# HySonLab/Protein_Redesign

Hardware: AMD Instinct MI355X
Metric: denoising-steps/sec (fwd+rev) per complex, N=256 res (higher is better)
Workload: dtype f32; 1 GPU; configs[1]: synthetic 256-residue + 64-atom ligand (N=320), single_dim=512 pair_dim=64 num_blocks=4 num_steps=1000, 1 complex/GPU, sharded by sample index (no data-path collective; one all_gather of the samples at the end of the timed region); samples_per_gpu=1, hip_graph=True, outputs_finite=True, backend=single process

## Files before the change

include/prd_hip.h:

```cpp
#ifndef PRD_HIP_H
#define PRD_HIP_H

#include <stddef.h>
#include <stdint.h>

#ifdef __cplusplus
extern "C" {
#endif

#ifndef __HIP__
typedef struct ihipStream_t* hipStream_t;
#endif

#define PRD_VERSION 101
#define PRD_STEP_BOUNDARY_SYNC_INTS 2
#define PRD_ERR_ARG (-1)
#define PRD_ERR_ALIGN (-2)
#define PRD_ERR_UNSUPPORTED (-3)
#define PRD_ERR_WORKSPACE (-4)

int prd_version(void);

#define PRD_ARITH_FP32 0
#define PRD_ARITH_SPLIT16 1
// ... 29 lines not shown
    int act, act_from;
    const float* addmat; long long sad1, sad2; int ldadd;
    const float* colmask; long long scm1; float fill;
    const float* rowmask; long long srm1;
    const float* mulmat; long long smu1, smu2; int ldmul;
    const float* resid; long long sr1, sr2; int ldr;
    int tile_hint;
    int a_ln;
    float* ln_out; int ldlo;
    int arith;
    float* C2; int ldc2; int n_split;
    int rowmask_cols;
    const float* rscale;
    float* ws; size_t ws_bytes;
    const float* wsum;
    float* out_ln; int ldol;
    float a_scale;
    int mul_pos;
    const unsigned* a_amax;
} PrdGemm;
size_t prd_gemm_slab_workspace(int M, int N, int K);
int prd_gemm_slab_ok(int M, int N, int K, int arith);
int prd_gemm(const PrdGemm* args, hipStream_t stream);

int prd_ln_rows(const float* x, float* y, const float* gamma, const float* beta,
                int rows, int C, int ldx, int ldy, hipStream_t stream);
int prd_softmax_rows(float* x, int rows, int n, int ld, hipStream_t stream);

int prd_static_pair(float* out, const float* atom_mask, const float* residue_mask, const float* bond_mask,
                    const int64_t* bond_feats, const int64_t* bond_distance,
                    const int64_t* residue_index, const int64_t* chain_index,
                    const float* tab_b0, const float* tab_b1, const float* tab_b2,
                    const float* tab_bdist, const float* tab_relpos,
                    int max_bond_distance, int max_relpos, int b, int N, int P, hipStream_t stream);
int prd_atom_embed(float* out, const int64_t* atom_feats, const float* atom_mask, const float* tables,
                   const int* offsets, int n_feats, int b, int N, int S, hipStream_t stream);
int prd_single_init(float* single, const float* static_single, const float* seq_t, const float* residue_mask,
                    const float* w_rt, int rows, int S, int n_cls, hipStream_t stream);
int prd_time_embed(float* ebeta, const int64_t* t, const float* freqs, const float* w_beta,
                   int num_steps, int b, int P, int time_dim, hipStream_t stream);
int prd_pair_init(float* pair, const float* static_pair, const float* z, const float* mask,
                  const float* centers, const float* w_dist, const float* ebeta,
                  int b, int N, int P, int dist_dim, int arith, hipStream_t stream);

int prd_pair_bias(float* bias_out, const float* pair, const float* gamma, const float* beta,
                  const float* w, const float* bvec, int b, int N, int P, int H, hipStream_t stream);
// ... 143 lines not shown
```

protein_redesign_amd/_lib.py:

```python
from __future__ import annotations

import ctypes as C
import os

import torch

HERE = os.path.dirname(os.path.abspath(__file__))
LIB_PATH = os.environ.get("PRD_LIB", os.path.join(HERE, "libprd_hip.so"))

vp, ci, cf, cz, cll = C.c_void_p, C.c_int, C.c_float, C.c_size_t, C.c_longlong


class PrdGemm(C.Structure):
    _fields_ = [
        ("A", vp), ("B", vp), ("C", vp),
        ("M", ci), ("N", ci), ("K", ci),
        ("lda", ci), ("ldb", ci), ("ldc", ci),
        ("G1", ci), ("G2", ci),
        ("sa1", cll), ("sa2", cll), ("sb1", cll), ("sb2", cll), ("sc1", cll), ("sc2", cll),
        ("b_kn", ci), ("alpha", cf), ("colscale", vp),
        ("bias", vp), ("act", ci), ("act_from", ci),
        ("addmat", vp), ("sad1", cll), ("sad2", cll), ("ldadd", ci),
        ("colmask", vp), ("scm1", cll), ("fill", cf),
        ("rowmask", vp), ("srm1", cll),
# ... 1 lines not shown
        ("resid", vp), ("sr1", cll), ("sr2", cll), ("ldr", ci),
        ("tile_hint", ci),
        ("a_ln", ci),
        ("ln_out", vp), ("ldlo", ci),
        ("arith", ci),
        ("C2", vp), ("ldc2", ci), ("n_split", ci),
        ("rowmask_cols", ci),
        ("rscale", vp),
        ("ws", vp), ("ws_bytes", cz),
        ("wsum", vp),
        ("out_ln", vp), ("ldol", ci),
        ("a_scale", cf),
        ("mul_pos", ci),
        ("a_amax", vp),
    ]


SIGNATURES = {
    "prd_version": [],
    "prd_tri_attn_variant": [ci, ci, ci],
    "prd_gemm": [C.POINTER(PrdGemm), vp],
    "prd_gemm_slab_workspace": [ci, ci, ci],
    "prd_gemm_slab_ok": [ci, ci, ci, ci],
    "prd_ln_rows": [vp, vp, vp, vp, ci, ci, ci, ci, vp],
    "prd_softmax_rows": [vp, ci, ci, ci, vp],
    "prd_static_pair": [vp] * 13 + [ci] * 5 + [vp],
    "prd_atom_embed": [vp] * 5 + [ci] * 4 + [vp],
    "prd_single_init": [vp] * 5 + [ci] * 3 + [vp],
    "prd_time_embed": [vp] * 4 + [ci] * 4 + [vp],
    "prd_pair_init": [vp] * 7 + [ci] * 5 + [vp],
    "prd_pair_bias": [vp] * 6 + [ci] * 4 + [vp],
    "prd_pair_bias2": [vp] * 6 + [ci] + [vp] * 5 + [ci] * 4 + [vp],
    "prd_opm_pair": [vp] * 6 + [ci] * 6 + [vp],
    "prd_pair_head_supported": [ci, ci, ci, ci],
    "prd_pair_head": [vp] * 7 + [ci] + [vp] * 3 + [ci, ci] + [vp] * 5 + [ci] + [vp] * 5 + [ci] * 5 + [vp],
    "prd_outer_linear": [vp] * 4 + [ci] + [vp] * 2 + [ci] * 5 + [vp, ci, vp],
    "prd_tri_mul": [vp] * 11 + [ci] * 5 + [vp, cz, vp, ci, vp],
    "prd_tri_mul_contract": [vp, vp, ci, ci, ci, ci, vp],
    "prd_tri_mul_contract_scaled": [vp, vp, vp, ci, ci, ci, ci, vp],
    "prd_tri_mul_chain_supported": [ci, ci, ci],
    "prd_tri_attn_core_fused_supported": [ci, ci, ci],
    "prd_tri_attn_core_fused": [vp] * 12 + [ci] * 6 + [vp],
    "prd_tri_mul_chain": [vp, vp, vp, vp, ci, ci, ci, vp, cz, ci, vp],
    "prd_tri_mul_out_bwd": [vp] * 15 + [ci] * 4 + [vp],
    "prd_tri_mul_out_bwd_amax": [vp] * 15 + [ci] * 4 + [vp, vp],
    "prd_tri_mul_bwd_operands": [vp, vp, ci, ci, ci, vp],
# ... 32 lines not shown
    "prd_tri_attn_v2_supported": [ci, ci, ci],
    "prd_tri_attn_out": [vp] * 5 + [ci] * 4 + [vp, ci, vp],
    "prd_spa_attn_core_supported": [ci, ci, ci],
    "prd_spa_attn_core_workspace": [ci, ci, ci, ci],
    "prd_spa_attn_core": [vp, vp, ci, vp, vp, ci, ci, ci, ci, vp, cz, ci, vp],
    "prd_workspace_bytes": [C.c_char_p, ci, ci, ci, ci],
    "prd_tri_attn_pair_supported": [ci, ci, ci],
    "prd_tri_attn_pair": [vp, vp, vp, vp, vp, ci, ci, ci, ci, ci, vp, ci, vp],
    "prd_tri_attn_heads_supported": [ci] * 5,
    "prd_tri_attn_heads_workspace_bytes": [ci] * 5,
    "prd_tri_attn_core_heads": [vp] * 8 + [ci] * 6 + [vp, cz, ci, vp],
    "prd_tri_attn_core_heads_lse": [vp] * 9 + [ci] * 6 + [vp, cz, ci, vp],
    "prd_tri_attn_bwd_heads_supported": [ci] * 5,
    "prd_tri_attn_bwd_heads_workspace_bytes": [ci] * 5,
    "prd_tri_attn_bwd_core_heads": [vp] * 12 + [ci] * 6 + [vp, cz, ci, vp],
}

GEMM_MODES = {"fp32": 0, "split16": 1, "bf16x3": 1}
DEFAULT_GEMM_MODE = "split16"

_ARITH_BEFORE_STREAM = ("prd_coord_head", "prd_pair_head", "prd_pair_init", "prd_opm_pair", "prd_outer_linear", "prd_tri_mul", "prd_tri_mul_contract", "prd_tri_mul_contract_scaled", "prd_tri_mul_proj_bwd",
                        "prd_tri_attn", "prd_tri_attn_core", "prd_tri_attn_out", "prd_pair_transition", "prd_block_tail", "prd_tri_mul_chain",
                        "prd_linear_wgrad", "prd_pair_linear", "prd_spa_attn_core", "prd_tri_attn_pair",
                        "prd_tri_attn_core_heads", "prd_tri_attn_core_heads_lse", "prd_tri_attn_bwd_core_heads")
_ARITH_LAST = ("prd_tri_attn_variant", "prd_tri_mul_chain_supported", "prd_tri_attn_core_fused_supported", "prd_tri_attn_stats_bytes",
               "prd_gemm_slab_ok", "prd_pair_head_supported", "prd_pair_linear_supported", "prd_spa_attn_core_supported",
               "prd_tri_attn_pair_supported", "prd_tri_attn_heads_supported",
               "prd_tri_attn_bwd_heads_supported")
_TUNE_BEFORE_STREAM = ("prd_tri_attn_core_v2", "prd_tri_attn_core_v2_lse")
_TUNE_LAST = ("prd_tri_attn_v2_supported", "prd_tri_attn_v2_form")


def tune_from_env(env=None) -> int:
    env = os.environ if env is None else env

    def geti(name, default):
        v = env.get(name)
        return default if v is None or v == "" else int(v)

    t = geti("PRD_TA_VARIANT", 0) & 15
    if geti("PRD_TA2_V3", 1) == 0:
        t |= 1 << 4
    if geti("PRD_TA2_LONG", 1) == 0:
        t |= 1 << 5
    f = geti("PRD_TA2_FLAGS", -1)
    if f >= 0:
        t |= (1 << 6) | ((f & 31) << 7)
    if geti("PRD_OL_VARIANT", 0) == 1:
        t |= 1 << 12
    nw = geti("PRD_TMS_NW", 8)
    t |= (1 << 13) if nw == 12 else (2 << 13) if nw == 16 else 0
# ... 168 lines not shown
```

protein_redesign_amd/csrc/prd_gemm.hip:

```cpp
#include "prd_common.h"
#include "../../include/prd_hip.h"
#include <mutex>

namespace {

constexpr int KC = 32;
constexpr int LDT = KC + 4;

PRD_DEV void epilogue_store(const PrdGemm& g, int g1, int g2, int m, int n, float v, float* __restrict__ C) {
    v = v * g.alpha;
    if (g.colscale) v *= g.colscale[n];
    if (g.bias) v += g.bias[n];
    if (g.addmat) v += g.addmat[g1 * g.sad1 + g2 * g.sad2 + (size_t)m * g.ldadd + n];
    if (g.colmask && g.colmask[g1 * g.scm1 + n] < 0.5f) v = g.fill;
    const int act = (n >= g.act_from) ? g.act : 0;
    if (act == 1) v = relu_nan(v);
    else if (act == 2) v = sigmoidf_(v);
    if (g.rowmask && (g.rowmask_cols <= 0 || n < g.rowmask_cols)) v *= g.rowmask[g1 * g.srm1 + m];
    if (g.mulmat) {
        const float mv = g.mulmat[g1 * g.smu1 + g2 * g.smu2 + (size_t)m * g.ldmul + n];
        v = g.mul_pos ? (mv > 0.f ? v : 0.f) : v * mv;
    }
    if (g.resid) {
        const float rv = g.resid[g1 * g.sr1 + g2 * g.sr2 + (size_t)m * g.ldr + n];
// ... 623 lines not shown
}

template <int D, int KG>
static int launch_ring(const PrdGemm& g, dim3 grid, hipStream_t stream) {
    const size_t lds = (size_t)KG * 2 * 4 * 32 * 64 * 2 + 1024;
    static std::once_flag once;
    std::call_once(once, [] {
        (void)hipFuncSetAttribute((const void*)gemm_ring_kernel<D, KG, true>, hipFuncAttributeMaxDynamicSharedMemorySize, 160 * 1024);
        (void)hipFuncSetAttribute((const void*)gemm_ring_kernel<D, KG, false>, hipFuncAttributeMaxDynamicSharedMemorySize, 160 * 1024);
    });
    if (g.a_ln) hipLaunchKernelGGL((gemm_ring_kernel<D, KG, true>), grid, dim3(256 * KG), lds, stream, g);
    else hipLaunchKernelGGL((gemm_ring_kernel<D, KG, false>), grid, dim3(256 * KG), lds, stream, g);
    return (int)hipGetLastError();
}

static int launch_ring_bkn(const PrdGemm& g, dim3 grid, hipStream_t stream) {
    const size_t lds = (size_t)2 * 4 * 32 * 64 * 2 + 1024;
    hipLaunchKernelGGL((gemm_ring_kernel<8, 1, false, true>), grid, dim3(256), lds, stream, g);
    return (int)hipGetLastError();
}

constexpr int SL_BM = 160, SL_BN = 64, SL_KS = 128, SL_NW = 10;
constexpr int SL_LDS = (SL_BM + SL_BN) * SL_KS * 4;
__global__ __launch_bounds__(SL_NW * 64) void gemm_slab_kernel(const float* __restrict__ A, const float* __restrict__ W,
                                                               float* __restrict__ ws, int M, int N, int K, int lda, int ldb,
                                                               int tiles_m, int tiles_n, int nslab, int spw, int xmap, float wscale) {
    extern __shared__ __attribute__((aligned(16))) unsigned char sl[];
    constexpr int APL = SL_BM * 256, WOFF = 2 * APL, WPL = SL_BN * 256;
    const int tid = threadIdx.x, lane = tid & 63, r = lane & 31, hi = lane >> 5;
    const int wave = __builtin_amdgcn_readfirstlane(tid >> 6);
    const int rt = wave >> 1, ct = wave & 1;
    const int SK = (nslab + spw - 1) / spw;
    int tile_m, tile_n, sg;
    if (xmap == 1) {
        const int xcd = blockIdx.x & 7, j = blockIdx.x >> 3, tiles = tiles_m * tiles_n;
        sg = xcd + 8 * (j / tiles);
        const int t_ = j % tiles;
        tile_m = t_ % tiles_m; tile_n = t_ / tiles_m;
    } else if (xmap == 2) {
        const int xcd = blockIdx.x & 7, j = blockIdx.x >> 3, tn_per = tiles_n / (8 / SK);
        sg = xcd % SK;
        tile_m = j % tiles_m; tile_n = (xcd / SK) * tn_per + j / tiles_m;
    } else {
        const int ncombo = tiles_m * SK, combo = blockIdx.x % ncombo;
        tile_n = blockIdx.x / ncombo; tile_m = combo % tiles_m; sg = combo / tiles_m;
    }
    const int m0 = tile_m * SL_BM, n0 = tile_n * SL_BN;
    const int prow = tid >> 5, piece = tid & 31;
    f32x16 acc;
#pragma unroll
    for (int q = 0; q < 16; ++q) acc[q] = 0.f;
    const int s_end = (sg + 1) * spw < nslab ? (sg + 1) * spw : nslab;
    for (int sl_i = sg * spw; sl_i < s_end; ++sl_i) {
        const prd_rsrc ra = make_rsrc(A + (size_t)m0 * lda + (size_t)sl_i * SL_KS), rb = make_rsrc(W + (size_t)n0 * ldb + (size_t)sl_i * SL_KS);
        u32x4 va[8], vb[4];
#pragma unroll
        for (int i = 0; i < 8; ++i) {
            const int row = prow + 20 * i;
            va[i] = __builtin_bit_cast(u32x4, __builtin_amdgcn_raw_buffer_load_b128(ra, (m0 + row < M) ? ((unsigned)row * lda + 4 * piece) * 4u : BUF_OOB, 0, 0));
        }
#pragma unroll
        for (int i = 0; i < 4; ++i) {
            const int row = prow + 20 * i;
            vb[i] = __builtin_bit_cast(u32x4, __builtin_amdgcn_raw_buffer_load_b128(rb, (row < SL_BN && n0 + row < N) ? ((unsigned)row * ldb + 4 * piece) * 4u : BUF_OOB, 0, 0));
        }
        if (sl_i > sg * spw) __syncthreads();
#pragma unroll
        for (int i = 0; i < 8; ++i) {
            const int row = prow + 20 * i;
            unsigned h0, l0, h1, l1;
            split2h(__uint_as_float(va[i][0]), __uint_as_float(va[i][1]), h0, l0);
            split2h(__uint_as_float(va[i][2]), __uint_as_float(va[i][3]), h1, l1);
            unsigned char* d_ = sl + row * 256 + (((piece >> 1) ^ (row & 15)) << 4) + (piece & 1) * 8;
            *reinterpret_cast<u32x2*>(d_) = u32x2{h0, h1};
            *reinterpret_cast<u32x2*>(d_ + APL) = u32x2{l0, l1};
        }
#pragma unroll
        for (int i = 0; i < 4; ++i) {
            const int row = prow + 20 * i;
            if (row < SL_BN) {
                unsigned h0, l0, h1, l1;
                split2h(wscale * __uint_as_float(vb[i][0]), wscale * __uint_as_float(vb[i][1]), h0, l0);
                split2h(wscale * __uint_as_float(vb[i][2]), wscale * __uint_as_float(vb[i][3]), h1, l1);
                unsigned char* d_ = sl + WOFF + row * 256 + (((piece >> 1) ^ (row & 15)) << 4) + (piece & 1) * 8;
                *reinterpret_cast<u32x2*>(d_) = u32x2{h0, h1};
                *reinterpret_cast<u32x2*>(d_ + WPL) = u32x2{l0, l1};
            }
        }
        __syncthreads();
        const unsigned char* ab = sl + (rt * 32 + r) * 256;
        const unsigned char* bb = sl + WOFF + (ct * 32 + r) * 256;
#pragma unroll
        for (int st = 0; st < SL_KS / 16; ++st) {
            const unsigned so = (unsigned)((2 * st + hi) ^ (r & 15)) << 4;
            const u32x4 ah = *reinterpret_cast<const u32x4*>(ab + so), al = *reinterpret_cast<const u32x4*>(ab + APL + so);
            const u32x4 bh = *reinterpret_cast<const u32x4*>(bb + so), bl = *reinterpret_cast<const u32x4*>(bb + WPL + so);
            acc = __builtin_amdgcn_mfma_f32_32x32x16_f16(__builtin_bit_cast(f16x8_t, ah), __builtin_bit_cast(f16x8_t, bh), acc, 0, 0, 0);
            acc = __builtin_amdgcn_mfma_f32_32x32x16_f16(__builtin_bit_cast(f16x8_t, ah), __builtin_bit_cast(f16x8_t, bl), acc, 0, 0, 0);
            acc = __builtin_amdgcn_mfma_f32_32x32x16_f16(__builtin_bit_cast(f16x8_t, al), __builtin_bit_cast(f16x8_t, bh), acc, 0, 0, 0);
        }
    }
    const int n = n0 + ct * 32 + r;
    if (n < N) {
        float* wp = ws + (size_t)sg * M * N + n;
        const float inv = 1.0f / wscale;
#pragma unroll
        for (int q = 0; q < 16; ++q) {
            const int m = m0 + rt * 32 + drow32(q, hi);
            if (m < M) wp[(size_t)m * N] = acc[q] * inv;
        }
    }
}

__global__ __launch_bounds__(128) void gemm_slab_reduce_kernel(PrdGemm g, const float* __restrict__ ws, int SK) {
    __shared__ float red[4];
    const int tid = threadIdx.x, lane = tid & 63, wave = tid >> 6;
    const int chunks = (g.N + 511) / 512;
    const int m = blockIdx.x / chunks, n = (blockIdx.x - m * chunks) * 512 + 4 * tid;
    const bool live = n < g.N;
// ... 40 lines not shown
        }
    }
    if (live) {
#pragma unroll
        for (int e = 0; e < 4; ++e) {
            float v = vv[e] * g.alpha;
            if (g.colscale) v *= g.colscale[n + e];
            if (g.bias) v += g.bias[n + e];
            const int act = (n + e >= g.act_from) ? g.act : 0;
            if (act == 1) v = relu_nan(v);
            else if (act == 2) v = sigmoidf_(v);
            if (g.rowmask && (g.rowmask_cols <= 0 || n + e < g.rowmask_cols)) v *= g.rowmask[m];
            if (g.resid) { const float rv = g.resid[(size_t)m * g.ldr + n + e]; v += g.rscale ? rv * g.rscale[n + e] : rv; }
            vv[e] = v;
        }
        if (g.C2 && n >= g.n_split) *reinterpret_cast<float4*>(g.C2 + (size_t)m * g.ldc2 + (n - g.n_split)) = make_float4(vv[0], vv[1], vv[2], vv[3]);
        else *reinterpret_cast<float4*>(g.C + (size_t)m * g.ldc + n) = make_float4(vv[0], vv[1], vv[2], vv[3]);
    }
    if (g.out_ln) {
        const float mu = block_sum(live ? (vv[0] + vv[1]) + (vv[2] + vv[3]) : 0.f) / (float)g.N;
        const float d0 = vv[0] - mu, d1 = vv[1] - mu, d2 = vv[2] - mu, d3 = vv[3] - mu;
        const float rz = 1.0f / sqrtf(block_sum(live ? (d0 * d0 + d1 * d1) + (d2 * d2 + d3 * d3) : 0.f) / (float)g.N + 1e-5f);
        if (live) *reinterpret_cast<float4*>(g.out_ln + (size_t)m * g.ldol + n) = make_float4(d0 * rz, d1 * rz, d2 * rz, d3 * rz);
    }
}

__global__ __launch_bounds__(256) void ln_rows_kernel(const float* __restrict__ x, float* __restrict__ y,
                                                      const float* __restrict__ gamma, const float* __restrict__ beta,
                                                      int rows, int C, int ldx, int ldy) {
    const int lane = threadIdx.x & 63;
    const int row = blockIdx.x * 4 + (threadIdx.x >> 6);
    if (row >= rows) return;
    const float* xr = x + (size_t)row * ldx;
    float s = 0.f;
    for (int c = lane; c < C; c += 64) s += xr[c];
    for (int o = 32; o > 0; o >>= 1) s += __shfl_xor(s, o);
    const float mean = s / C;
    float v = 0.f;
    for (int c = lane; c < C; c += 64) { const float d = xr[c] - mean; v += d * d; }
    for (int o = 32; o > 0; o >>= 1) v += __shfl_xor(v, o);
    const float rstd = 1.0f / sqrtf(v / C + 1e-5f);
    float* yr = y + (size_t)row * ldy;
    for (int c = lane; c < C; c += 64) {
        float t = (xr[c] - mean) * rstd;
        if (gamma) t = t * gamma[c] + beta[c];
        yr[c] = t;
// ... 24 lines not shown
    float* xr = x + (size_t)row * ld;
    float m = -INFINITY;
    for (int c = lane; c < n; c += 64) m = fmaxf(m, xr[c]);
    for (int o = 32; o > 0; o >>= 1) m = fmaxf(m, __shfl_xor(m, o));
    float s = 0.f;
    for (int c = lane; c < n; c += 64) s += expf(xr[c] - m);
    for (int o = 32; o > 0; o >>= 1) s += __shfl_xor(s, o);
    for (int c = lane; c < ld; c += 64) xr[c] = (c < n) ? expf(xr[c] - m) / s : 0.f;
}

bool slab_plan(int M, int N, int K, int arith_full, int* tiles_m, int* tiles_n, int* nslab, int* spw) {
    if (arith_full < 0 || (arith_full & 0xff) != PRD_ARITH_SPLIT16 || ((arith_full >> 8) & (1 << 16))) return false;
    if (M < 96 || N <= 0 || K <= 0 || (K % SL_KS) || (N % 4)) return false;
    *tiles_m = prd_ceil_div(M, SL_BM);
    *tiles_n = prd_ceil_div(N, SL_BN);
    *nslab = K / SL_KS;
    const long tiles = (long)*tiles_m * *tiles_n;
    if (tiles * *nslab < 128 || tiles > 4096) return false;
    int s = 1;
    while (tiles * prd_ceil_div(*nslab, s) > 512 && s < *nslab) ++s;
    *spw = s;
    return true;
}
}

extern "C" int prd_gemm_slab_ok(int M, int N, int K, int arith) {
    int a, b, c, d;
    return slab_plan(M, N, K, arith, &a, &b, &c, &d) ? 1 : 0;
}

extern "C" int prd_gemm(const PrdGemm* args, hipStream_t stream) {
    const PrdGemm& g = *args;
    if (!g.A || !g.B || !g.C || g.M <= 0 || g.N <= 0 || g.K <= 0 || g.G1 <= 0 || g.G2 <= 0) return PRD_ERR_ARG;
    if (g.arith < 0 || (g.arith & 0xff) > 1) return PRD_ERR_ARG;
    const int arith = g.arith & 0xff;
    if ((g.lda & 3) || (g.ldb & 3)) return PRD_ERR_ALIGN;
    const int batches = g.G1 * g.G2;
    if (g.ln_out && (!g.a_ln || batches != 1 || (g.ldlo & 3) || g.ldlo < g.K)) return PRD_ERR_ARG;
    if (g.C2 && (batches != 1 || g.n_split <= 0 || g.n_split >= g.N || g.ldc2 < g.N - g.n_split)) return PRD_ERR_ARG;
    const long tiles64 = (long)prd_ceil_div(g.M, 64) * prd_ceil_div(g.N, 64) * batches;
    if (g.ws && g.tile_hint == 0 && !g.b_kn && batches == 1 && !g.addmat && !g.colmask && !g.mulmat &&
        (!g.C2 || ((g.n_split & 3) == 0 && (g.ldc2 & 3) == 0 && !g.out_ln)) && (!g.ln_out || (g.wsum && (g.K & 3) == 0)) &&
        (!g.a_ln || g.wsum) && (!g.out_ln || (g.N <= 512 && (g.ldol & 3) == 0)) && (g.ldc & 3) == 0 && (!g.resid || (g.ldr & 3) == 0)) {
        int tiles_m, tiles_n, nslab, spw;
        if (slab_plan(g.M, g.N, g.K, g.arith, &tiles_m, &tiles_n, &nslab, &spw)) {
            const int SK = prd_ceil_div(nslab, spw);
            if ((size_t)SK * g.M * g.N * sizeof(float) > g.ws_bytes) return PRD_ERR_WORKSPACE;
            static std::once_flag once;
            std::call_once(once, [] { (void)hipFuncSetAttribute((const void*)gemm_slab_kernel, hipFuncAttributeMaxDynamicSharedMemorySize, 160 * 1024); });
            const int xmap = (SK % 8 == 0) ? 1 : ((SK < 8 && 8 % SK == 0 && tiles_n % (8 / SK) == 0) ? 2 : 0);
            hipLaunchKernelGGL(gemm_slab_kernel, dim3((unsigned)(tiles_m * tiles_n * SK)), dim3(SL_NW * 64), SL_LDS, stream, g.A, g.B, g.ws, g.M, g.N,
                               g.K, g.lda, g.ldb, tiles_m, tiles_n, nslab, spw, xmap, H2_WSCALE);
            hipLaunchKernelGGL(gemm_slab_reduce_kernel, dim3((unsigned)(g.M * prd_ceil_div(g.N, 512))), dim3(128), 0, stream, g, g.ws, SK);
            return (int)hipGetLastError();
        }
    }
    if (g.out_ln) return PRD_ERR_UNSUPPORTED;
    if (arith == PRD_ARITH_SPLIT16 && g.tile_hint == 0 && !g.b_kn && (g.K % 32) == 0 && tiles64 >= 512 && g.G1 * g.G2 == 1 &&
        (!g.a_ln || (g.K % 16) == 0)) {
        dim3 grid(prd_ceil_div(g.M, 64) * prd_ceil_div(g.N, 64), batches);
        PrdGemm gx = g;
        if (g.N >= 512 && (long)g.N > 2L * g.M && ((g.arith >> 8) & (1 << 18))) {
            gx.tile_hint = -8;
            grid.x = 8u * prd_ceil_div(g.M, 64) * prd_ceil_div(prd_ceil_div(g.N, 64), 8);
        }
        static std::once_flag once1, once4;
        if (g.K >= 1024) {
            const size_t lds = (size_t)4 * 2 * 4 * 64 * 64 + 512;
            std::call_once(once4, [] { (void)hipFuncSetAttribute((const void*)gemm_h2_kernel<4>, hipFuncAttributeMaxDynamicSharedMemorySize, 160 * 1024); });
            hipLaunchKernelGGL((gemm_h2_kernel<4>), grid, dim3(1024), lds, stream, gx);
        } else {
            const size_t lds = (size_t)2 * 4 * 64 * 64 + 512;
            std::call_once(once1, [] { (void)hipFuncSetAttribute((const void*)gemm_h2_kernel<1>, hipFuncAttributeMaxDynamicSharedMemorySize, 160 * 1024); });
            hipLaunchKernelGGL((gemm_h2_kernel<1>), grid, dim3(256), lds, stream, gx);
        }
// ... 74 lines not shown
```

protein_redesign_amd/ops.py:

```python
from __future__ import annotations

import math
import os
from typing import Mapping, Optional, Tuple

import torch

from ._lib import PrdGemm, arithmetic, check, dptr, lib, stream

F32 = torch.float32


_QUEUES = {}


def task_queue(device) -> int:
    import os
    if not os.environ.get("PRD_TASK_QUEUE"):
        return 0
    key = torch.device(device).index if torch.device(device).index is not None else torch.cuda.current_device()
    q = _QUEUES.get(key)
    if q is None:
        q = _QUEUES[key] = torch.zeros(256, dtype=torch.int32, device=f"cuda:{key}")
    return q.data_ptr()
# ... 793 lines not shown


SPA_CORE = os.environ.get("PRD_SPA_CORE", "1") != "0"


def pack_attention(wq, wk, wv, wg, bg, q_scale: float):
    HC = wq.shape[0]
    w = torch.cat([wq, wk, wv, wg], dim=0).contiguous()
    bias = torch.cat([torch.zeros(3 * HC, device=w.device, dtype=F32), bg]).contiguous()
    colscale = torch.cat([torch.full((HC,), q_scale, device=w.device, dtype=F32),
                          torch.ones(3 * HC, device=w.device, dtype=F32)]).contiguous()
    return w, bias, colscale


def project_qkvg(x_normed, packed, HC: int, ln_a: bool = False) -> torch.Tensor:
    b, N, S = x_normed.shape
    w, pbias, colscale = packed
    L = 4 * HC
    qkvg = torch.empty(b, N, L, device=x_normed.device, dtype=F32)
    gemm(x_normed, w, qkvg, b * N, L, S, S, S, L, bias=pbias, colscale=colscale, act=2, act_from=3 * HC, a_ln=ln_a)
    return qkvg


def gated_attention_single(x_normed, mask, bias, packed, wo, bo, H: int, c: int, *,
                           key_mask: bool, resid: Optional[torch.Tensor], ln_a: bool = False,
                           qkvg: Optional[torch.Tensor] = None, rscale: Optional[torch.Tensor] = None,
                           out_ln: Optional[torch.Tensor] = None, logits_fp32: bool = True) -> torch.Tensor:
    b, N, S = x_normed.shape
    HC = H * c
    w, pbias, colscale = packed
    L = 4 * HC
    if qkvg is None:
        if ln_a and not ln_fusable(S):
            x_normed, ln_a = layer_norm(x_normed.contiguous()), False
        qkvg = project_qkvg(x_normed, packed, HC, ln_a)
    o = torch.empty(b, N, HC, device=x_normed.device, dtype=F32)
    if c == 16 and HC == 64:
        qp, ldq = row_block(qkvg)
        check(lib().prd_single_attn_core(dptr(o), qp, ldq, dptr(bias), dptr(mask) if key_mask else None,
                                         b, N, H, c, stream()), "prd_single_attn_core")
        return linear(o, wo, bo, resid=resid, rscale=rscale)
    if SPA_CORE and not logits_fp32 and lib().prd_spa_attn_core_supported(N, c) == 1:
        qp, ldq = row_block(qkvg)
        nws = int(lib().prd_spa_attn_core_workspace(b, N, H, c))
        wsb = torch.empty(max(nws // 4, 4), device=o.device, dtype=F32)
        check(lib().prd_spa_attn_core(dptr(o), qp, ldq, dptr(bias), dptr(mask) if key_mask else None, b, N, H, c, dptr(wsb), nws, stream()),
              "prd_spa_attn_core")
        return linear(o, wo, bo, resid=resid, rscale=rscale, slab=slab_ok(b * N, wo.shape[0], HC), out_ln=out_ln)
    ldp = round_up(N, 4)
    logits = torch.empty(b, H, N, ldp, device=x_normed.device, dtype=F32)
    qkvg, L = row_block(qkvg)
    gemm(qkvg, qkvg, logits, N, N, c, L, L, ldp, b_off=HC, G1=b, G2=H, sa=(N * L, c), sb=(N * L, c),
         sc=(H * N * ldp, N * ldp), addmat=bias, sad=(H * N * N, N * N), ldadd=N,
         colmask=(mask if key_mask else None), scm1=N, fill=-(2.0 ** 15),
         tile_hint=32 if logits_fp32 else 0)
    pv = dict(b_off=2 * HC, G1=b, G2=H, sa=(H * N * ldp, N * ldp), sb=(N * L, c), sc=(N * HC, c), b_kn=True, mulmat=qkvg, mul_off=3 * HC,
              smu=(N * L, c), ldmul=L, a_scale=1024.0)
    if ldp != N or gemm(logits, qkvg, o, N, c, N, ldp, L, HC, a_ln=2, unsupported_ok=True, **pv) is None:
        softmax_rows_(logits, N)
        gemm(logits, qkvg, o, N, c, N, ldp, L, HC, **pv)
    return linear(o, wo, bo, resid=resid, rscale=rscale, slab=slab_ok(b * N, wo.shape[0], HC), out_ln=out_ln)


def project_many(single, packed, P_first: int, *, act: int, act_from: int, xhat=None):
# ... 2 lines not shown
    Ncat = w.shape[0]
    out = torch.empty(b, N, Ncat, device=single.device, dtype=F32)
    if xhat is not None:
        gemm(xhat, w, out, b * N, Ncat, S, S, S, Ncat, bias=pbias, colscale=colscale, act=act, act_from=act_from)
        return xhat, out
    if ln_fusable(S):
        x = torch.empty_like(single)
        gemm(single, w, out, b * N, Ncat, S, S, S, Ncat, bias=pbias, colscale=colscale, act=act, act_from=act_from, a_ln=True, ln_out=x)
    else:
        x = layer_norm(single)
        gemm(x, w, out, b * N, Ncat, S, S, S, Ncat, bias=pbias, colscale=colscale, act=act, act_from=act_from)
    return x, out


def transition_single(single, w1, b1, w2, b2, *, residual: bool, wsum1=None, want_ln: bool = False):
    b, N, S = single.shape
    Hd = w1.shape[0]
    slab1 = wsum1 is not None and slab_ok(b * N, Hd, S)
    slab2 = slab_ok(b * N, S, Hd)
    h = linear(single, w1, b1, act=1, ln_a=True, slab=slab1, wsum=wsum1 if slab1 else None)
    xhat = torch.empty_like(single) if (want_ln and slab2 and S <= 512) else None
    out = linear(h, w2, b2, resid=single if residual else None, slab=slab2, out_ln=xhat)
    return (out, xhat) if want_ln else out
```

protein_redesign_amd/trunk.py:

```python
from __future__ import annotations

import os

import math
from argparse import Namespace
from typing import Mapping, Optional, Tuple

import torch
from torch import nn

from . import ops
from .af2_blocks import OuterProductUpdate, SPAttention

_VARIANCE_INITS = {
    "default": (1.0, "fan_in", "truncated_normal"),
    "relu": (2.0, "fan_in", "truncated_normal"),
    "glorot": (1.0, "fan_avg", "uniform"),
    "normal": (1.0, "fan_in", "normal"),
}
_TRUNC_STD_CORRECTION = 0.87962566103423978


def _variance_scaling_(weight: torch.Tensor, scale: float, mode: str, distribution: str) -> None:
    fan_out, fan_in = weight.shape
# ... 98 lines not shown
        self.ab_proj = Linear(pair_dim, pair_dim * 2, init="default")
        self.ab_gate = Linear(pair_dim, pair_dim * 2, init="gating")
        self.ab_norm = nn.LayerNorm(pair_dim, elementwise_affine=False)
        self.out_proj = Linear(pair_dim, pair_dim, init="final")
        self.out_gate = Linear(pair_dim, pair_dim, init="gating")

    def weights(self):
        return (self.ab_proj.weight, self.ab_proj.bias, self.ab_gate.weight, self.ab_gate.bias,
                self.out_proj.weight, self.out_proj.bias, self.out_gate.weight, self.out_gate.bias)

    def run(self, pair, mask, *, residual: bool, out=None, ws=None):
        return ops.tri_mul(pair, mask, self.weights(), incoming=self.mode == "incoming", residual=residual, out=out, ws=ws)

    def forward(self, pair: torch.Tensor, mask_2d: torch.Tensor) -> torch.Tensor:
        return self.run(pair.contiguous(), _node_mask(mask_2d), residual=False)


_TRI_MUL_CHAIN = os.environ.get("PRD_TRI_MUL_CHAIN", "1") != "0"
_TRI_ATTN_FUSE = os.environ.get("PRD_TRI_ATTN_FUSE", "0") == "1"
_PAIR_HEAD = os.environ.get("PRD_PAIR_HEAD", "1") != "0"
_MERGE_HEAD = os.environ.get("PRD_MERGE_HEAD", "1") != "0"
_HEAD_SLAB = os.environ.get("PRD_HEAD_SLAB", "0") == "1"
_MERGE_PROJ = os.environ.get("PRD_MERGE_PROJ", "1") != "0"


class OuterLinear(nn.Module):

    def __init__(self, single_dim: int, pair_dim: int):
        super().__init__()
        self.single_dim, self.pair_dim = single_dim, pair_dim
        self.norm = nn.LayerNorm(single_dim, elementwise_affine=False)
        self.linear = Linear(single_dim * 2, pair_dim, init="final")

    def run(self, single, pair, *, residual: bool, out=None):
        b, N, S = single.shape
        w = self.linear.weight
        u = torch.empty(b, N, self.pair_dim, device=single.device, dtype=torch.float32)
        if ops.ln_fusable(S):
            x = torch.empty_like(single)
            ops.gemm(single, w, u, b * N, self.pair_dim, S, S, 2 * S, self.pair_dim, b_off=S, a_ln=True, ln_out=x)
        else:
            x = ops.layer_norm(single)
            ops.gemm(x, w, u, b * N, self.pair_dim, S, S, 2 * S, self.pair_dim, b_off=S)
        return ops.outer_linear_pair(pair, x, u, w, self.linear.bias, residual=residual, out=out)

    def forward(self, x: torch.Tensor) -> torch.Tensor:
# ... 39 lines not shown
    def _after_transition_pack(self, next_block, tail):
        S, P = self.outer_linear.single_dim, self.outer_linear.pair_dim
        w_ol = self.outer_linear.linear.weight
        if next_block is not None:
            sa = next_block.single_attn
            ws = (w_ol, *sa.weights()[:5])

            def build():
                w, pb, cs = sa.packed()
                dev = w.device
                return (torch.cat([w_ol[:, S:], w]).contiguous(), torch.cat([torch.zeros(P, device=dev), pb]).contiguous(),
                        torch.cat([torch.ones(P, device=dev), cs]).contiguous())
            return ops.cached_pack(self, "after_transition_next", ws, build), 2, P + 3 * sa.num_heads * sa.head_dim
        if tail is not None:
            tw, tb = tail
            ws = (w_ol, tw, tb)

            def build():
                dev = tw.device
                return (torch.cat([w_ol[:, S:], tw]).contiguous(), torch.cat([torch.zeros(P, device=dev), tb]).contiguous(), None)
            return ops.cached_pack(self, "after_transition_tail", ws, build), 1, P
        return None, 0, 0

    def run_(self, single: torch.Tensor, pair: torch.Tensor, mask: torch.Tensor, ws=None, bias=None, next_block=None, spare_holder=None,
             qkvg=None, tail=None, extra=None):
        sa = self.single_attn
        b, N = mask.shape
        ta = self.pair_attn_ending.attn
        general = not ops.default_head_layout(ta.num_heads, ta.head_dim)
        if general and pair.is_cuda:
            ops.check_head_layout(ta.num_heads, ta.head_dim, pair.shape[-1])
        if ws is None:
            ws = torch.empty(ws_floats(b, N, pair.shape[-1], ta.num_heads, ta.head_dim), device=pair.device, dtype=torch.float32)
        if bias is None:
            bias = ops.pair_bias(pair, self.attn_bias[1].weight, self.attn_bias[1].bias)
        single = sa.run_single(single, mask, bias, single, ln_a=True, qkvg=qkvg)
        fc = self.single_fc
        wsum1 = ops.cached_pack(self, "fc1_rowsum", (fc[1].weight,), lambda: fc[1].weight.double().sum(1).float().contiguous())
        single, xhat = ops.transition_single(single, fc[1].weight, fc[1].bias, fc[3].weight, fc[3].bias, residual=True, wsum1=wsum1,
                                             want_ln=True)
        packed, act, act_from = self._after_transition_pack(next_block if extra is not None else None, tail if extra is not None else None)
        if packed is not None and _MERGE_PROJ:
            P = self.outer_linear.pair_dim
            x, cat = ops.project_many(single, packed, P, act=act, act_from=act_from, xhat=xhat)
            ol = self.outer_linear.linear
            ops.outer_linear_pair(pair, x, cat[..., :P], ol.weight, ol.bias, residual=True, out=pair)
            extra["qkvg" if next_block is not None else "tail"] = cat[..., P:]
        else:
            self.outer_linear.run(single, pair, residual=True, out=pair)
        if _TRI_MUL_CHAIN and ops.tri_mul_chain_supported(N, pair.shape[-1]):
            ops.tri_mul_chain_(pair, mask, self.pair_mul_outgoing.weights(), self.pair_mul_incoming.weights(), ws=ws)
        else:
            self.pair_mul_outgoing.run(pair, mask, residual=True, out=pair, ws=ws)
            self.pair_mul_incoming.run(pair, mask, residual=True, out=pair, ws=ws)
        pf = self.pair_fc
        nb_w = next_block.attn_bias[1].weight if next_block is not None else None
        nb_b = next_block.attn_bias[1].bias if next_block is not None else None
        if general:
            self.pair_attn_starting.run(pair, mask, residual=True, out=pair, ws=ws)
            og = ops.tri_attn_core_heads(pair, mask, ta.weights()[:5], ta.num_heads, ta.head_dim, ending=True, ws=ws)
            if og.shape[-1] == 64:
                next_bias = ops.block_tail_(pair, og, ta.out_proj.weight, ta.out_proj.bias, pf[1].weight, pf[1].bias,
                                            pf[3].weight, pf[3].bias, nb_w, nb_b)
            else:
                ops.linear(og, ta.out_proj.weight, ta.out_proj.bias, resid=pair, out=pair)
                ops.pair_transition(pair, pf[1].weight, pf[1].bias, pf[3].weight, pf[3].bias, residual=True, out=pair)
                next_bias = ops.pair_bias(pair, nb_w, nb_b) if nb_w is not None else None
            return single, pair, next_bias
        nog = b * N * N * 64
        if _TRI_ATTN_FUSE and ops.tri_attn_core_fused_supported(N, pair.shape[-1]) and ws.numel() >= 2 * nog:
# ... 144 lines not shown
```

Baseline: 567.0 denoising-steps/s.

## Fold single-attention out-projection into fc1 GEMM with fused LN reduce

Precomputes W1·Wo and W1·bo so the first transition GEMM consumes the attention output directly as extra K columns, instead of running a separate out-projection linear and materialising the updated single. A new reduce kernel sums the slab partials, recomputes the residual single and its LayerNorm statistics per row, and applies the LN correction algebraically using row sums of W1 before ReLU. This removes one GEMM launch and a round trip of the single activation. In exchange it adds a templated slab kernel path, extra LDS, and a folded weight product whose rounding differs slightly from the unfolded computation.

```diff
diff --git a/include/prd_hip.h b/include/prd_hip.h
--- a/include/prd_hip.h
+++ b/include/prd_hip.h
@@ -75,6 +75,11 @@
 size_t prd_gemm_slab_workspace(int M, int N, int K);
 int prd_gemm_slab_ok(int M, int N, int K, int arith);
 int prd_gemm(const PrdGemm* args, hipStream_t stream);
+
+int prd_single_fc1_folded_ok(int M, int S, int HC, int Hd, int arith);
+int prd_single_fc1_folded(const float* single, const float* og, const float* w1cat, const float* woT, const float* bo,
+                          const float* wsum1, const float* w1bo, const float* b1, float* single_out, float* h,
+                          int M, int S, int HC, int Hd, float* ws, size_t ws_bytes, int arith, hipStream_t stream);
 
 int prd_ln_rows(const float* x, float* y, const float* gamma, const float* beta,
                 int rows, int C, int ldx, int ldy, hipStream_t stream);
diff --git a/protein_redesign_amd/_lib.py b/protein_redesign_amd/_lib.py
--- a/protein_redesign_amd/_lib.py
+++ b/protein_redesign_amd/_lib.py
@@ -47,6 +47,8 @@
     "prd_gemm": [C.POINTER(PrdGemm), vp],
     "prd_gemm_slab_workspace": [ci, ci, ci],
     "prd_gemm_slab_ok": [ci, ci, ci, ci],
+    "prd_single_fc1_folded_ok": [ci] * 5,
+    "prd_single_fc1_folded": [vp] * 10 + [ci] * 4 + [vp, cz, ci, vp],
     "prd_ln_rows": [vp, vp, vp, vp, ci, ci, ci, ci, vp],
     "prd_softmax_rows": [vp, ci, ci, ci, vp],
     "prd_static_pair": [vp] * 13 + [ci] * 5 + [vp],
@@ -125,11 +127,11 @@
 _ARITH_BEFORE_STREAM = ("prd_coord_head", "prd_pair_head", "prd_pair_init", "prd_opm_pair", "prd_outer_linear", "prd_tri_mul", "prd_tri_mul_contract", "prd_tri_mul_contract_scaled", "prd_tri_mul_proj_bwd",
                         "prd_tri_attn", "prd_tri_attn_core", "prd_tri_attn_out", "prd_pair_transition", "prd_block_tail", "prd_tri_mul_chain",
                         "prd_linear_wgrad", "prd_pair_linear", "prd_spa_attn_core", "prd_tri_attn_pair",
-                        "prd_tri_attn_core_heads", "prd_tri_attn_core_heads_lse", "prd_tri_attn_bwd_core_heads")
+                        "prd_tri_attn_core_heads", "prd_tri_attn_core_heads_lse", "prd_tri_attn_bwd_core_heads", "prd_single_fc1_folded")
 _ARITH_LAST = ("prd_tri_attn_variant", "prd_tri_mul_chain_supported", "prd_tri_attn_core_fused_supported", "prd_tri_attn_stats_bytes",
                "prd_gemm_slab_ok", "prd_pair_head_supported", "prd_pair_linear_supported", "prd_spa_attn_core_supported",
                "prd_tri_attn_pair_supported", "prd_tri_attn_heads_supported",
-               "prd_tri_attn_bwd_heads_supported")
+               "prd_tri_attn_bwd_heads_supported", "prd_single_fc1_folded_ok")
 _TUNE_BEFORE_STREAM = ("prd_tri_attn_core_v2", "prd_tri_attn_core_v2_lse")
 _TUNE_LAST = ("prd_tri_attn_v2_supported", "prd_tri_attn_v2_form")
 
diff --git a/protein_redesign_amd/csrc/prd_gemm.hip b/protein_redesign_amd/csrc/prd_gemm.hip
--- a/protein_redesign_amd/csrc/prd_gemm.hip
+++ b/protein_redesign_amd/csrc/prd_gemm.hip
@@ -669,11 +669,14 @@
 
 constexpr int SL_BM = 160, SL_BN = 64, SL_KS = 128, SL_NW = 10;
 constexpr int SL_LDS = (SL_BM + SL_BN) * SL_KS * 4;
+template <int EX>
 __global__ __launch_bounds__(SL_NW * 64) void gemm_slab_kernel(const float* __restrict__ A, const float* __restrict__ W,
                                                                float* __restrict__ ws, int M, int N, int K, int lda, int ldb,
-                                                               int tiles_m, int tiles_n, int nslab, int spw, int xmap, float wscale) {
+                                                               int tiles_m, int tiles_n, int nslab, int spw, int xmap, float wscale,
+                                                               const float* __restrict__ A2, int lda2) {
     extern __shared__ __attribute__((aligned(16))) unsigned char sl[];
     constexpr int APL = SL_BM * 256, WOFF = 2 * APL, WPL = SL_BN * 256;
+    constexpr int XOFF = SL_LDS, XROW = 32 * (EX > 0 ? EX : 1), XPL = (SL_BM + SL_BN) * XROW, XQ = 4 * (EX > 0 ? EX : 1);
     const int tid = threadIdx.x, lane = tid & 63, r = lane & 31, hi = lane >> 5;
     const int wave = __builtin_amdgcn_readfirstlane(tid >> 6);
     const int rt = wave >> 1, ct = wave & 1;
@@ -698,6 +701,17 @@
 #pragma unroll
     for (int q = 0; q < 16; ++q) acc[q] = 0.f;
     const int s_end = (sg + 1) * spw < nslab ? (sg + 1) * spw : nslab;
+    u32x4 xa[EX > 0 ? EX : 1], xb;
+    if (EX > 0) {
+        const prd_rsrc r2 = make_rsrc(A2 + (size_t)m0 * lda2 + (size_t)sg * 16 * EX), rw = make_rsrc(W + (size_t)n0 * ldb + K + (size_t)sg * 16 * EX);
+#pragma unroll
+        for (int i = 0; i < EX; ++i) {
+            const int idx = tid + SL_NW * 64 * i, row = idx / XQ, q = idx - row * XQ;
+            xa[i] = __builtin_bit_cast(u32x4, __builtin_amdgcn_raw_buffer_load_b128(r2, (m0 + row < M) ? ((unsigned)row * lda2 + 4 * q) * 4u : BUF_OOB, 0, 0));
+        }
+        const int row = tid / XQ, q = tid - row * XQ;
+        xb = __builtin_bit_cast(u32x4, __builtin_amdgcn_raw_buffer_load_b128(rw, (row < SL_BN && n0 + row < N) ? ((unsigned)row * ldb + 4 * q) * 4u : BUF_OOB, 0, 0));
+    }
     for (int sl_i = sg * spw; sl_i < s_end; ++sl_i) {
         const prd_rsrc ra = make_rsrc(A + (size_t)m0 * lda + (size_t)sl_i * SL_KS), rb = make_rsrc(W + (size_t)n0 * ldb + (size_t)sl_i * SL_KS);
         u32x4 va[8], vb[4];
@@ -712,6 +726,27 @@
             vb[i] = __builtin_bit_cast(u32x4, __builtin_amdgcn_raw_buffer_load_b128(rb, (row < SL_BN && n0 + row < N) ? ((unsigned)row * ldb + 4 * piece) * 4u : BUF_OOB, 0, 0));
         }
         if (sl_i > sg * spw) __syncthreads();
+        if (EX > 0 && sl_i == sg * spw) {
+#pragma unroll
+            for (int i = 0; i < EX; ++i) {
+                const int idx = tid + SL_NW * 64 * i, row = idx / XQ, q = idx - row * XQ;
+                unsigned h0, l0, h1, l1;
+                split2h(__uint_as_float(xa[i][0]), __uint_as_float(xa[i][1]), h0, l0);
+                split2h(__uint_as_float(xa[i][2]), __uint_as_float(xa[i][3]), h1, l1);
+                unsigned char* d_ = sl + XOFF + row * XROW + (q >> 1) * 16 + (q & 1) * 8;
+                *reinterpret_cast<u32x2*>(d_) = u32x2{h0, h1};
+                *reinterpret_cast<u32x2*>(d_ + XPL) = u32x2{l0, l1};
+            }
+            const int row = tid / XQ, q = tid - row * XQ;
+            if (row < SL_BN) {
+                unsigned h0, l0, h1, l1;
+                split2h(wscale * __uint_as_float(xb[0]), wscale * __uint_as_float(xb[1]), h0, l0);
+                split2h(wscale * __uint_as_float(xb[2]), wscale * __uint_as_float(xb[3]), h1, l1);
+                unsigned char* d_ = sl + XOFF + (SL_BM + row) * XROW + (q >> 1) * 16 + (q & 1) * 8;
+                *reinterpret_cast<u32x2*>(d_) = u32x2{h0, h1};
+                *reinterpret_cast<u32x2*>(d_ + XPL) = u32x2{l0, l1};
+            }
+        }
 #pragma unroll
         for (int i = 0; i < 8; ++i) {
             const int row = prow + 20 * i;
@@ -742,6 +777,18 @@
             const unsigned so = (unsigned)((2 * st + hi) ^ (r & 15)) << 4;
             const u32x4 ah = *reinterpret_cast<const u32x4*>(ab + so), al = *reinterpret_cast<const u32x4*>(ab + APL + so);
             const u32x4 bh = *reinterpret_cast<const u32x4*>(bb + so), bl = *reinterpret_cast<const u32x4*>(bb + WPL + so);
+            acc = __builtin_amdgcn_mfma_f32_32x32x16_f16(__builtin_bit_cast(f16x8_t, ah), __builtin_bit_cast(f16x8_t, bh), acc, 0, 0, 0);
+            acc = __builtin_amdgcn_mfma_f32_32x32x16_f16(__builtin_bit_cast(f16x8_t, ah), __builtin_bit_cast(f16x8_t, bl), acc, 0, 0, 0);
+            acc = __builtin_amdgcn_mfma_f32_32x32x16_f16(__builtin_bit_cast(f16x8_t, al), __builtin_bit_cast(f16x8_t, bh), acc, 0, 0, 0);
+        }
+    }
+    if (EX > 0) {
+        const unsigned char* ab = sl + XOFF + (rt * 32 + r) * XROW + hi * 16;
+        const unsigned char* bb = sl + XOFF + (SL_BM + ct * 32 + r) * XROW + hi * 16;
+#pragma unroll
+        for (int st = 0; st < EX; ++st) {
+            const u32x4 ah = *reinterpret_cast<const u32x4*>(ab + 32 * st), al = *reinterpret_cast<const u32x4*>(ab + XPL + 32 * st);
+            const u32x4 bh = *reinterpret_cast<const u32x4*>(bb + 32 * st), bl = *reinterpret_cast<const u32x4*>(bb + XPL + 32 * st);
             acc = __builtin_amdgcn_mfma_f32_32x32x16_f16(__builtin_bit_cast(f16x8_t, ah), __builtin_bit_cast(f16x8_t, bh), acc, 0, 0, 0);
             acc = __builtin_amdgcn_mfma_f32_32x32x16_f16(__builtin_bit_cast(f16x8_t, ah), __builtin_bit_cast(f16x8_t, bl), acc, 0, 0, 0);
             acc = __builtin_amdgcn_mfma_f32_32x32x16_f16(__builtin_bit_cast(f16x8_t, al), __builtin_bit_cast(f16x8_t, bh), acc, 0, 0, 0);
@@ -828,6 +875,65 @@
         const float d0 = vv[0] - mu, d1 = vv[1] - mu, d2 = vv[2] - mu, d3 = vv[3] - mu;
         const float rz = 1.0f / sqrtf(block_sum(live ? (d0 * d0 + d1 * d1) + (d2 * d2 + d3 * d3) : 0.f) / (float)g.N + 1e-5f);
         if (live) *reinterpret_cast<float4*>(g.out_ln + (size_t)m * g.ldol + n) = make_float4(d0 * rz, d1 * rz, d2 * rz, d3 * rz);
+    }
+}
+
+template <int HC>
+__global__ __launch_bounds__(1024) void fc1_fold_reduce_kernel(const float* __restrict__ ws, int SK, int M, int N, int S,
+                                                               const float* __restrict__ single, const float* __restrict__ og,
+                                                               const float* __restrict__ woT, const float* __restrict__ bo,
+                                                               const float* __restrict__ wsum1, const float* __restrict__ w1bo,
+                                                               const float* __restrict__ b1, float* __restrict__ single_out,
+                                                               float* __restrict__ h) {
+    __shared__ float red[16];
+    const int tid = threadIdx.x, lane = tid & 63, wave = tid >> 6, nwave = blockDim.x >> 6;
+    const int m = blockIdx.x, n = 4 * tid;
+    const bool live = n < N, own = tid < S;
+    float4 sum = make_float4(0.f, 0.f, 0.f, 0.f);
+    const float* wp = ws + (size_t)m * N + (live ? n : 0);
+    const size_t sstride = (size_t)M * N;
+    for (int s0 = 0; s0 < SK; s0 += 4) {
+        float4 v[4];
+#pragma unroll
+        for (int j = 0; j < 4; ++j) v[j] = *reinterpret_cast<const float4*>(wp + (size_t)(s0 + j < SK ? s0 + j : 0) * sstride);
+#pragma unroll
+        for (int j = 0; j < 4; ++j)
+            if (s0 + j < SK) { sum.x += v[j].x; sum.y += v[j].y; sum.z += v[j].z; sum.w += v[j].w; }
+    }
+    const float* ogr = og + (size_t)m * HC;
+    const float* wc = woT + (own ? tid : 0);
+    const float s0 = own ? single[(size_t)m * S + tid] : 0.f, b0 = own ? bo[tid] : 0.f;
+    float p[4] = {0.f, 0.f, 0.f, 0.f};
+    float wv[HC];
+#pragma unroll
+    for (int j = 0; j < HC; ++j) wv[j] = wc[(size_t)j * S];
+    __builtin_amdgcn_sched_barrier(0);
+#pragma unroll
+    for (int j = 0; j < HC; j += 4) {
+#pragma unroll
+        for (int e = 0; e < 4; ++e) p[e] = fmaf(ogr[j + e], wv[j + e], p[e]);
+    }
+    const float sp = own ? s0 + (((p[0] + p[1]) + (p[2] + p[3])) + b0) : 0.f;
+    auto block_sum = [&](float x) {
+#pragma unroll
+        for (int o = 32; o > 0; o >>= 1) x += __shfl_xor(x, o);
+        __syncthreads();
+        if (lane == 0) red[wave] = x;
+        __syncthreads();
+        float t = 0.f;
+        for (int w = 0; w < nwave; ++w) t += red[w];
+        return t;
+    };
+    const float mu = block_sum(sp) / (float)S;
+    const float d = own ? sp - mu : 0.f;
+    const float rz = 1.0f / sqrtf(block_sum(d * d) / (float)S + 1e-5f);
+    if (own) single_out[(size_t)m * S + tid] = sp;
+    if (live) {
+        const float4 cs = *reinterpret_cast<const float4*>(wsum1 + n), cw = *reinterpret_cast<const float4*>(w1bo + n);
+        const float4 cb = *reinterpret_cast<const float4*>(b1 + n);
+        const float v0 = ((sum.x + cw.x) - mu * cs.x) * rz + cb.x, v1 = ((sum.y + cw.y) - mu * cs.y) * rz + cb.y;
+        const float v2 = ((sum.z + cw.z) - mu * cs.z) * rz + cb.z, v3 = ((sum.w + cw.w) - mu * cs.w) * rz + cb.w;
+        *reinterpret_cast<float4*>(h + (size_t)m * N + n) = make_float4(relu_nan(v0), relu_nan(v1), relu_nan(v2), relu_nan(v3));
     }
 }
 
@@ -898,6 +1004,47 @@
     *spw = s;
     return true;
 }
+int slab_xmap(int SK, int tiles_n) { return (SK % 8 == 0) ? 1 : ((SK < 8 && 8 % SK == 0 && tiles_n % (8 / SK) == 0) ? 2 : 0); }
+
+bool fc1_fold_plan(int M, int S, int HC, int Hd, int arith_full, int* tiles_m, int* tiles_n, int* nslab, int* spw, int* ex) {
+    if (HC != 64 || S > 512 || Hd > 4096 || 128 * prd_ceil_div(Hd, 512) < S) return false;
+    if (!slab_plan(M, Hd, S, arith_full, tiles_m, tiles_n, nslab, spw)) return false;
+    const int SK = prd_ceil_div(*nslab, *spw);
+    if (HC % (16 * SK)) return false;
+    *ex = HC / (16 * SK);
+    return *ex == 1;
+}
+}
+
+extern "C" int prd_single_fc1_folded_ok(int M, int S, int HC, int Hd, int arith) {
+    int a, b, c, d, e;
+    return fc1_fold_plan(M, S, HC, Hd, arith, &a, &b, &c, &d, &e) ? 1 : 0;
+}
+
+extern "C" int prd_single_fc1_folded(const float* single, const float* og, const float* w1cat, const float* woT, const float* bo,
+                                     const float* wsum1, const float* w1bo, const float* b1, float* single_out, float* h,
+                                     int M, int S, int HC, int Hd, float* ws, size_t ws_bytes, int arith, hipStream_t stream) {
+    if (!single || !og || !w1cat || !woT || !bo || !wsum1 || !w1bo || !b1 || !single_out || !h || !ws || M <= 0 || S <= 0 || HC <= 0 || Hd <= 0)
+        return PRD_ERR_ARG;
+    if (arith < 0 || (arith & 0xff) > 1) return PRD_ERR_ARG;
+    int tiles_m, tiles_n, nslab, spw, ex;
+    if (!fc1_fold_plan(M, S, HC, Hd, arith, &tiles_m, &tiles_n, &nslab, &spw, &ex)) return PRD_ERR_UNSUPPORTED;
+    const uintptr_t al = reinterpret_cast<uintptr_t>(single) | reinterpret_cast<uintptr_t>(og) | reinterpret_cast<uintptr_t>(w1cat) |
+                         reinterpret_cast<uintptr_t>(wsum1) | reinterpret_cast<uintptr_t>(w1bo) | reinterpret_cast<uintptr_t>(b1) |
+                         reinterpret_cast<uintptr_t>(h) | reinterpret_cast<uintptr_t>(ws);
+    if (al & 15) return PRD_ERR_ALIGN;
+    const int SK = prd_ceil_div(nslab, spw);
+    if ((size_t)SK * M * Hd * sizeof(float) > ws_bytes) return PRD_ERR_WORKSPACE;
+    static std::once_flag once;
+    std::call_once(once, [] { (void)hipFuncSetAttribute((const void*)gemm_slab_kernel<1>, hipFuncAttributeMaxDynamicSharedMemorySize, 160 * 1024); });
+    const int xmap = slab_xmap(SK, tiles_n);
+    const dim3 grid((unsigned)(tiles_m * tiles_n * SK));
+    const size_t lds = SL_LDS + (size_t)(SL_BM + SL_BN) * 32 * ex * 2;
+    hipLaunchKernelGGL(gemm_slab_kernel<1>, grid, dim3(SL_NW * 64), lds, stream, single, w1cat, ws, M, Hd, S, S, S + HC, tiles_m, tiles_n, nslab,
+                       spw, xmap, H2_WSCALE, og, HC);
+    hipLaunchKernelGGL(fc1_fold_reduce_kernel<64>, dim3((unsigned)M), dim3(128 * prd_ceil_div(Hd, 512)), 0, stream, ws, SK, M, Hd, S, single, og, woT,
+                       bo, wsum1, w1bo, b1, single_out, h);
+    return (int)hipGetLastError();
 }
 
 extern "C" int prd_gemm_slab_ok(int M, int N, int K, int arith) {
@@ -923,10 +1070,10 @@
             const int SK = prd_ceil_div(nslab, spw);
             if ((size_t)SK * g.M * g.N * sizeof(float) > g.ws_bytes) return PRD_ERR_WORKSPACE;
             static std::once_flag once;
-            std::call_once(once, [] { (void)hipFuncSetAttribute((const void*)gemm_slab_kernel, hipFuncAttributeMaxDynamicSharedMemorySize, 160 * 1024); });
-            const int xmap = (SK % 8 == 0) ? 1 : ((SK < 8 && 8 % SK == 0 && tiles_n % (8 / SK) == 0) ? 2 : 0);
-            hipLaunchKernelGGL(gemm_slab_kernel, dim3((unsigned)(tiles_m * tiles_n * SK)), dim3(SL_NW * 64), SL_LDS, stream, g.A, g.B, g.ws, g.M, g.N,
-                               g.K, g.lda, g.ldb, tiles_m, tiles_n, nslab, spw, xmap, H2_WSCALE);
+            std::call_once(once, [] { (void)hipFuncSetAttribute((const void*)gemm_slab_kernel<0>, hipFuncAttributeMaxDynamicSharedMemorySize, 160 * 1024); });
+            const int xmap = slab_xmap(SK, tiles_n);
+            hipLaunchKernelGGL(gemm_slab_kernel<0>, dim3((unsigned)(tiles_m * tiles_n * SK)), dim3(SL_NW * 64), SL_LDS, stream, g.A, g.B, g.ws, g.M, g.N,
+                               g.K, g.lda, g.ldb, tiles_m, tiles_n, nslab, spw, xmap, H2_WSCALE, (const float*)nullptr, 0);
             hipLaunchKernelGGL(gemm_slab_reduce_kernel, dim3((unsigned)(g.M * prd_ceil_div(g.N, 512))), dim3(128), 0, stream, g, g.ws, SK);
             return (int)hipGetLastError();
         }
diff --git a/protein_redesign_amd/ops.py b/protein_redesign_amd/ops.py
--- a/protein_redesign_amd/ops.py
+++ b/protein_redesign_amd/ops.py
@@ -839,6 +839,15 @@
     return qkvg
 
 
+def single_attn_core(qkvg, mask, bias, H: int, c: int) -> torch.Tensor:
+    b, N = qkvg.shape[:2]
+    o = torch.empty(b, N, H * c, device=qkvg.device, dtype=F32)
+    qp, ldq = row_block(qkvg)
+    check(lib().prd_single_attn_core(dptr(o), qp, ldq, dptr(bias), dptr(mask) if mask is not None else None,
+                                     b, N, H, c, stream()), "prd_single_attn_core")
+    return o
+
+
 def gated_attention_single(x_normed, mask, bias, packed, wo, bo, H: int, c: int, *,
                            key_mask: bool, resid: Optional[torch.Tensor], ln_a: bool = False,
                            qkvg: Optional[torch.Tensor] = None, rscale: Optional[torch.Tensor] = None,
@@ -851,12 +860,10 @@
         if ln_a and not ln_fusable(S):
             x_normed, ln_a = layer_norm(x_normed.contiguous()), False
         qkvg = project_qkvg(x_normed, packed, HC, ln_a)
+    if c == 16 and HC == 64:
+        o = single_attn_core(qkvg, mask if key_mask else None, bias, H, c)
+        return linear(o, wo, bo, resid=resid, rscale=rscale)
     o = torch.empty(b, N, HC, device=x_normed.device, dtype=F32)
-    if c == 16 and HC == 64:
-        qp, ldq = row_block(qkvg)
-        check(lib().prd_single_attn_core(dptr(o), qp, ldq, dptr(bias), dptr(mask) if key_mask else None,
-                                         b, N, H, c, stream()), "prd_single_attn_core")
-        return linear(o, wo, bo, resid=resid, rscale=rscale)
     if SPA_CORE and not logits_fp32 and lib().prd_spa_attn_core_supported(N, c) == 1:
         qp, ldq = row_block(qkvg)
         nws = int(lib().prd_spa_attn_core_workspace(b, N, H, c))
@@ -905,3 +912,29 @@
     xhat = torch.empty_like(single) if (want_ln and slab2 and S <= 512) else None
     out = linear(h, w2, b2, resid=single if residual else None, slab=slab2, out_ln=xhat)
     return (out, xhat) if want_ln else out
+
+
+def fc1_fold_ok(M: int, S: int, HC: int, Hd: int) -> bool:
+    return lib().prd_single_fc1_folded_ok(M, S, HC, Hd) == 1
+
+
+def pack_fc1_fold(wo, bo, w1):
+    w1d, wod = w1.detach().double(), wo.detach().double()
+    w1cat = torch.cat([w1.detach().float(), (w1d @ wod).float()], dim=1).contiguous()
+    return w1cat, wo.detach().t().contiguous(), w1d.sum(1).float().contiguous(), (w1d @ bo.detach().double()).float().contiguous()
+
+
+def transition_single_folded(single, og, pack, bo, b1, w2, b2, *, want_ln: bool = False):
+    b, N, S = single.shape
+    w1cat, woT, wsum1, w1bo = pack
+    Hd, HC = w1cat.shape[0], og.shape[-1]
+    M = b * N
+    s1 = torch.empty_like(single)
+    h = torch.empty(b, N, Hd, device=single.device, dtype=F32)
+    wsb = gemm_workspace(single.device, int(lib().prd_gemm_slab_workspace(M, Hd, S)))
+    check(lib().prd_single_fc1_folded(dptr(single), dptr(og), dptr(w1cat), dptr(woT), dptr(bo), dptr(wsum1), dptr(w1bo), dptr(b1),
+                                      dptr(s1), dptr(h), M, S, HC, Hd, dptr(wsb), wsb.numel() * 4, stream()), "prd_single_fc1_folded")
+    slab2 = slab_ok(M, S, Hd)
+    xhat = torch.empty_like(single) if (want_ln and slab2 and S <= 512) else None
+    out = linear(h, w2, b2, resid=s1, slab=slab2, out_ln=xhat)
+    return (out, xhat) if want_ln else out
diff --git a/protein_redesign_amd/trunk.py b/protein_redesign_amd/trunk.py
--- a/protein_redesign_amd/trunk.py
+++ b/protein_redesign_amd/trunk.py
@@ -144,6 +144,7 @@
 _MERGE_HEAD = os.environ.get("PRD_MERGE_HEAD", "1") != "0"
 _HEAD_SLAB = os.environ.get("PRD_HEAD_SLAB", "0") == "1"
 _MERGE_PROJ = os.environ.get("PRD_MERGE_PROJ", "1") != "0"
+_FOLD_OUT_PROJ = os.environ.get("PRD_FOLD_OUT_PROJ", "1") != "0"
 
 
 class OuterLinear(nn.Module):
@@ -229,6 +230,31 @@
             return ops.cached_pack(self, "after_transition_tail", ws, build), 1, P
         return None, 0, 0
 
+    def single_track_(self, single, mask, bias, next_block=None, qkvg=None, tail=None, extra=None):
+        sa = self.single_attn
+        b, N, S = single.shape
+        fc = self.single_fc
+        HC, Hd = sa.num_heads * sa.head_dim, fc[1].weight.shape[0]
+        if _FOLD_OUT_PROJ and single.is_cuda and sa.head_dim == 16 and ops.fc1_fold_ok(b * N, S, HC, Hd):
+            if qkvg is None:
+                qkvg = ops.project_qkvg(single, sa.packed(), HC, ln_a=True)
+            og = ops.single_attn_core(qkvg, mask, bias, sa.num_heads, sa.head_dim)
+            wo, bo = sa.out_proj.weight, sa.out_proj.bias
+            pack = ops.cached_pack(self, "fc1_fold", (wo, bo, fc[1].weight), lambda: ops.pack_fc1_fold(wo, bo, fc[1].weight))
+            single, xhat = ops.transition_single_folded(single, og, pack, bo, fc[1].bias, fc[3].weight, fc[3].bias, want_ln=True)
+        else:
+            single = sa.run_single(single, mask, bias, single, ln_a=True, qkvg=qkvg)
+            wsum1 = ops.cached_pack(self, "fc1_rowsum", (fc[1].weight,), lambda: fc[1].weight.double().sum(1).float().contiguous())
+            single, xhat = ops.transition_single(single, fc[1].weight, fc[1].bias, fc[3].weight, fc[3].bias, residual=True, wsum1=wsum1,
+                                                 want_ln=True)
+        packed, act, act_from = self._after_transition_pack(next_block if extra is not None else None, tail if extra is not None else None)
+        if packed is None or not _MERGE_PROJ:
+            return single, None, None
+        P = self.outer_linear.pair_dim
+        x, cat = ops.project_many(single, packed, P, act=act, act_from=act_from, xhat=xhat)
+        extra["qkvg" if next_block is not None else "tail"] = cat[..., P:]
+        return single, x, cat[..., :P]
+
     def run_(self, single: torch.Tensor, pair: torch.Tensor, mask: torch.Tensor, ws=None, bias=None, next_block=None, spare_holder=None,
              qkvg=None, tail=None, extra=None):
         sa = self.single_attn
@@ -241,18 +267,10 @@
             ws = torch.empty(ws_floats(b, N, pair.shape[-1], ta.num_heads, ta.head_dim), device=pair.device, dtype=torch.float32)
         if bias is None:
             bias = ops.pair_bias(pair, self.attn_bias[1].weight, self.attn_bias[1].bias)
-        single = sa.run_single(single, mask, bias, single, ln_a=True, qkvg=qkvg)
-        fc = self.single_fc
-        wsum1 = ops.cached_pack(self, "fc1_rowsum", (fc[1].weight,), lambda: fc[1].weight.double().sum(1).float().contiguous())
-        single, xhat = ops.transition_single(single, fc[1].weight, fc[1].bias, fc[3].weight, fc[3].bias, residual=True, wsum1=wsum1,
-                                             want_ln=True)
-        packed, act, act_from = self._after_transition_pack(next_block if extra is not None else None, tail if extra is not None else None)
-        if packed is not None and _MERGE_PROJ:
-            P = self.outer_linear.pair_dim
-            x, cat = ops.project_many(single, packed, P, act=act, act_from=act_from, xhat=xhat)
+        single, x, u = self.single_track_(single, mask, bias, next_block=next_block, qkvg=qkvg, tail=tail, extra=extra)
+        if u is not None:
             ol = self.outer_linear.linear
-            ops.outer_linear_pair(pair, x, cat[..., :P], ol.weight, ol.bias, residual=True, out=pair)
-            extra["qkvg" if next_block is not None else "tail"] = cat[..., P:]
+            ops.outer_linear_pair(pair, x, u, ol.weight, ol.bias, residual=True, out=pair)
         else:
             self.outer_linear.run(single, pair, residual=True, out=pair)
         if _TRI_MUL_CHAIN and ops.tri_mul_chain_supported(N, pair.shape[-1]):
```

Result: faster. 572.9 denoising-steps/s, median of 6 (+1.0%).
